# MDFahimAnjum/AliasFree-Diffusion-Models-PyTorch

Hardware: AMD Instinct MI355X
Metric: train_step_images_per_sec (higher is better)
Workload: dtype f32; 1 GPU; CIFAR-10 32x32x3 synthetic, UNet variant=3 (Config D), batch 256/GPU, T=1000, AdamW lr 3e-4, random-init weights (seed 42); global_batch=256, parallelism=dp1, hip_graph=True, launch_mode=lanes

## Files before the change

aliasfree-diffusion-models-pytorch_amd/_lib.py:

```python
import ctypes
import os
import re

_PKG = os.path.dirname(os.path.abspath(__file__))
_ROOT = os.path.dirname(_PKG)
HEADER = os.path.join(_ROOT, "include", "afd.h")
LIBPATH = os.environ.get("AFD_LIBPATH") or os.path.join(_PKG, "libafd_hip.so")

_CTYPES = {
    "int": ctypes.c_int, "long": ctypes.c_long, "float": ctypes.c_float, "double": ctypes.c_double,
    "size_t": ctypes.c_size_t,
}
_DECL = re.compile(r"^(int|size_t|const char\*)\s+(afd_\w+)\s*\(([^;]*?)\)\s*;", re.M | re.S)


def _strip_comments(src):
    return re.sub(r"/\*.*?\*/", " ", src, flags=re.S)


def parse_header(path=HEADER):
    out = {}
    for ret, name, args in _DECL.findall(_strip_comments(open(path).read())):
        argtypes = []
        args = " ".join(args.split())
        if args not in ("", "void"):
            for a in args.split(","):
                a = a.strip()
                if "*" in a or a.startswith("afd_stream_t"):
                    argtypes.append(ctypes.c_void_p)
                else:
                    base = a.split()[0] if not a.startswith("unsigned") else a
                    argtypes.append(_CTYPES[base])
        restype = {"int": ctypes.c_int, "size_t": ctypes.c_size_t, "const char*": ctypes.c_char_p}[ret]
        out[name] = (restype, argtypes)
    return out


_VALUE_RETURNING = {"afd_device_count", "afd_tok_supported", "afd_conv3x3_weight_kinds", "afd_conv_wgrad_form",
                    "afd_grad_sqnorm_n_partials"}


class AfdError(RuntimeError):
    pass


class _Lib:
    def __init__(self):
        if not os.path.exists(LIBPATH):
            raise AfdError(
                f"{LIBPATH} not found: build it with `python -c 'import __graft_entry__ as g; g.build()'` "
                "(hipcc --offload-arch=gfx950). There is no CPU/eager fallback.")
        self.cdll = ctypes.CDLL(LIBPATH)
        self.sigs = parse_header()
        for name, (restype, argtypes) in self.sigs.items():
            fn = getattr(self.cdll, name)
            fn.restype, fn.argtypes = restype, argtypes
            if restype is ctypes.c_int and name not in _VALUE_RETURNING:
                setattr(self, name, self._checked(name, fn))
            else:
                setattr(self, name, fn)

# ... 21 lines not shown
```

aliasfree-diffusion-models-pytorch_amd/csrc/bf3_wgrad.hip:

```cpp
#include <algorithm>
#include <cstdint>
#include <cstdlib>
#include "common.h"
#include "bf3_weights.h"

namespace afd {

using f32x4 = __attribute__((ext_vector_type(4))) float;
using u32x4 = __attribute__((ext_vector_type(4))) uint32_t;

template <int S, int BN_, int BK_> struct BwGeo {
  static constexpr int TP = 128, G8 = S / 8;
  static constexpr int IPT = S * S >= TP ? 1 : TP / (S * S);
  static constexpr int R = S * S >= TP ? TP / S : S;
  static constexpr int TPI = S * S >= TP ? S * S / TP : 1;
  static constexpr int IG = (R + 2) * G8, NG = IPT * IG;
  static constexpr int BK = BK_, BN = BN_;
  static constexpr int NR = (BN / 16) * (BK / 32), NSG = 8 / NR;
  static constexpr int TASKS = (BK / 16) * NG * 16, NE = (TASKS + 511) / 512;
  static constexpr int PIECE = (BK / 16) * NG * 16;
};

__device__ __forceinline__ uint32_t bf_pack(__bf16 lo, __bf16 hi) {
  return (uint32_t)__builtin_bit_cast(uint16_t, lo) | ((uint32_t)__builtin_bit_cast(uint16_t, hi) << 16);
// ... 426 lines not shown
  }
  float* ps = part + (long)blockIdx.x * 27 * N;
#pragma unroll
  for (int j = 0; j < 4; ++j)
#pragma unroll
    for (int t = 0; t < 27; ++t) {
      const float v = wave_sum_to_lane63(acc[j][t]);
      if (lane == 63) ps[((long)(t / 3) * N + n0 + j) * 3 + (t % 3)] = v;
    }
}

static int g_wgbf3_mode = 0;
void wgrad_bf3_set_mode(int m) { g_wgbf3_mode = m; }

static void wgrad_bf3_tile(int Cin, int Cout, long nt, int* bn, int* bk) {
  static const int force = [] { const char* e = getenv("AFD_WGB_TILE"); return e ? atoi(e) : 0; }();
  const bool can = Cout % 64 == 0 && Cin % 64 == 0;
  const bool big = force ? force >= 64 : nt * (Cout / 64) * (Cin / 64) >= 1024;
  if (can && big) { *bn = 64; *bk = 64; return; }
  *bn = (Cout % 64 == 0 && Cin % 64 && (force ? force >= 64 : true)) ? 64 : 32;
  *bk = (Cin % 64 == 0 && Cout % 64 && (force ? force >= 64 : true)) ? 64 : 32;
}

void wgrad_bf3_tile_for(int Cin, int Cout, long nt, int* bn, int* bk) { wgrad_bf3_tile(Cin, Cout, nt, bn, bk); }
static int g_wg_arith_bf3 = 0;
void wgrad_arith_set(int m) { g_wg_arith_bf3 = m; }
bool wgrad_arith_is_bf3() { return g_wg_arith_bf3 != 0; }

static long g_wgb_target = 256;
void wgrad_plan_target_set(long wgs) { g_wgb_target = wgs; }

int wgrad_bf3_plan(int B, int Cin, int Cout, int H, int W, int* tps, int* ntiles) {
  if (g_wgbf3_mode == 1) return 0;
  if (H != W || (W != 4 && W != 8 && W != 16 && W != 32)) return 0;
  if (Cin % 32 || Cout % 32) return 0;
  if ((long)B * H * W * (Cin > Cout ? Cin : Cout) >= (1L << 31)) return 0;
  const long nt = W == 4 ? (B + 7) / 8 : (W == 8 ? (B + 1) / 2 : (long)B * (H * W / 128));
  int BN, BK;
  wgrad_bf3_tile(Cin, Cout, W == 4 ? (B + 7) / 8 : (W == 8 ? (B + 1) / 2 : (long)B * (H * W / 128)), &BN, &BK);
  const long blocks = (long)(Cout / BN) * (Cin / BK);
  static const long env_target = [] { const char* e = getenv("AFD_WGB_TARGET"); return e ? atol(e) : 0L; }();
  const long target = env_target > 0 ? env_target : g_wgb_target;
  long s = target / blocks;
  if (s < 1) s = 1;
  if (s > nt) s = nt;
  const long c = (nt + s - 1) / s;
  if (g_wgbf3_mode != 2 && nt * blocks < 128) return 0;
  *tps = (int)c; *ntiles = (int)nt;
  return (int)((nt + c - 1) / c);
}

template <int S, int BN, int BK>
static void wgrad_bf3_launch_t(const float* x, const float* dy, float* part, int B, int Cin, int Cout, int tps, int nt, int splits,
                               hipStream_t s) {
  using G = BwGeo<S, BN, BK>;
  const size_t lds = std::max((size_t)3 * G::PIECE * 16, G::NSG > 1 ? sizeof(float) * G::NR * 72 * 64 : (size_t)0);
  (void)lds_opt_in(&wgrad_bf3<S, BN, BK>, lds);
  hipLaunchKernelGGL((wgrad_bf3<S, BN, BK>), dim3((unsigned)splits, (unsigned)((Cout / BN) * (Cin / BK))), dim3(512), lds, s, x, dy,
                     part, B, Cin, Cout, tps, nt);
}

template <int BN, int BK>
static void wgrad_bf3_s4_launch_t(const float* x, const float* dy, float* part, int B, int Cin, int Cout, int tps, int nt, int splits,
                                  hipStream_t s) {
  constexpr int NR = (BN / 16) * (BK / 32);
  const size_t lds = std::max((size_t)3 * (BK / 16) * 40 * 16 * 16, 8 / NR > 1 ? sizeof(float) * NR * 72 * 64 : (size_t)0);
  (void)lds_opt_in(&wgrad_bf3_s4<BN, BK>, lds);
  hipLaunchKernelGGL((wgrad_bf3_s4<BN, BK>), dim3((unsigned)splits, (unsigned)((Cout / BN) * (Cin / BK))), dim3(512), lds, s, x, dy, part, B,
                     Cin, Cout, tps, nt);
}

int wgrad_bf3(const float* x, const float* dy, float* part, int B, int Cin, int Cout, int H, int W, hipStream_t s) {
// ... 76 lines not shown
```

aliasfree-diffusion-models-pytorch_amd/csrc/conv.hip:

```cpp
#include <cstdlib>
#include <algorithm>
#include "common.h"

namespace afd {

using f32x16 = __attribute__((ext_vector_type(16))) float;

static inline int gs_grid(long total, int block = 256) {
  long g = (total + block - 1) / block;
  return (int)(g < 1 ? 1 : (g > 65536 ? 65536 : g));
}

template <int KS>
__global__ void conv_direct_fwd(const float* __restrict__ x, const float* __restrict__ w, const float* __restrict__ bias,
                                const float* __restrict__ res, float* __restrict__ y,
                                int Cin, int Cout, int H, int W, int act, long total) {
  constexpr int T = KS * KS, R = KS / 2;
  for (long i = blockIdx.x * (long)blockDim.x + threadIdx.x; i < total; i += (long)gridDim.x * blockDim.x) {
    const int xx = i % W, yy = (i / W) % H;
    const long bc = i / ((long)W * H);
    const int co = bc % Cout; const long b = bc / Cout;
    float acc = bias ? bias[co] : 0.f;
    for (int ci = 0; ci < Cin; ++ci) {
      const float* xp = x + (b * Cin + ci) * (long)H * W;
// ... 699 lines not shown
  }
  return fold_launch(d, nd, s);
}

bool pw_launch(const float* in, const float* w, const float* bias, const float* res, float* out, int B, int K, int N, int P,
               int act, bool dgrad, hipStream_t s);
void pw_set_mode(int m);
int wino_plan(int B, int K, int N, int H, int W);
int wino_conv(const float* x, const float* w, const float* bias, const float* res, float* y, float* U, int B, int K, int N, int H,
               int W, int act, bool dgrad, bool weights_ready, hipStream_t s);
void wino_set_mode(int m);
void wino_weights_launch(const float* w, float* Uf, float* Ud, int Cin, int Cout, int kinds, hipStream_t s);
bool bf3_ok(int B, int K, int N, int H, int W);
void bf3_set_mode(int m);
void direct_form_set(int m);
bool direct_form_is_bf3();
void h2_sk_set_mode(int m);
void h2_lds_set(int m);
void h2_skw_set(int m);
void wino_weights_batched_launch(const afd_wino_desc* descs, const int* wg_desc, int n_wg, hipStream_t s);
void wino_set_grid(int g);
int wgrad_wino_plan(int B, int Cin, int Cout, int H, int W, int* bn, int* bk, int* cps, int* nchunks);
int wgrad_bf3_plan(int B, int Cin, int Cout, int H, int W, int* tps, int* ntiles);
int wgrad_bf3(const float* x, const float* dy, float* part, int B, int Cin, int Cout, int H, int W, hipStream_t s);
void wgrad_bf3_set_mode(int m);
void wgrad_arith_set(int m);
void wgrad_plan_target_set(long wgs);
bool wgrad_arith_is_bf3();
int wgrad_h2(const float* x, const float* dy, float* part, int B, int Cin, int Cout, int H, int W, hipStream_t s);
int pw_wgrad_h2(const float* x, const float* dy, float* part, float* bias_part, int B, int Cin, int Cout, int L, hipStream_t s);
bool ends_fwd(const float* x, const float* w, const float* bias, const float* res, float* y, int B, int Cin, int Cout, int H, int W,
              int ksize, int act, hipStream_t s);
bool ends_dgrad(const float* dy, const float* w, float* dx, int B, int Cin, int Cout, int H, int W, int ksize, hipStream_t s);
void ends_set_mode(int m);
int wgrad_cin3_plan(int B, int Cin, int Cout, int H, int W);
int wgrad_cin3(const float* x, const float* dy, float* part, int B, int Cin, int Cout, int H, int W, hipStream_t s);
void pw_wgrad_bf3_set_mode(int m);
int pw_wgrad_bf3_plan(int B, int Cin, int Cout, int L, int* sps, int* nsteps, int* nr, int* nt);
int pw_wgrad_bf3(const float* x, const float* dy, float* part, float* bias_part, int B, int Cin, int Cout, int L, hipStream_t s);
int wgrad_wino(const float* x, const float* dy, float* part, int B, int Cin, int Cout, int H, int W, hipStream_t s);
void wgrad_wino_set_mode(int m);

static inline bool use_mfma(int K, int N, int H, int W, int PT) { return N >= 8 && tile_ok(H, W, PT); }

static int g_conv_path = 0;

template <int T, bool DGRAD>
static int launch_mfma(const float* x, const float* w, const float* bias, const float* res, float* y,
                       int B, int K, int N, int H, int W, int act, hipStream_t s) {
  constexpr int KC = (T == 9) ? 8 : 32;
// ... 73 lines not shown
  else
    hipLaunchKernelGGL((conv_wgrad_mfma<T, WNn, WCn, NPB, 4>), grid, dim3(256), lds, s, x, dy, part, bias_part, B, Cin, Cout, H, W, p.cps, p.nchunks, g);
}

template <int T, int NPB>
static void launch_wgrad_roles(const float* x, const float* dy, float* part, float* bp, int B, int Cin, int Cout, int H, int W,
                               const WgradPlan& p, const TileGeom& g, hipStream_t s) {
  if (p.wnn == 2 && p.wcn == 2) launch_wgrad<T, 2, 2, NPB>(x, dy, part, bp, B, Cin, Cout, H, W, p, g, s);
  else if (p.wnn == 2) launch_wgrad<T, 2, 1, NPB>(x, dy, part, bp, B, Cin, Cout, H, W, p, g, s);
  else if (p.wcn == 2) launch_wgrad<T, 1, 2, NPB>(x, dy, part, bp, B, Cin, Cout, H, W, p, g, s);
  else launch_wgrad<T, 1, 1, NPB>(x, dy, part, bp, B, Cin, Cout, H, W, p, g, s);
}

}
using namespace afd;

extern "C" {

int afd_debug_conv_path(int mode) {
  if (mode >= 92 && mode <= 93) { ends_set_mode(mode - 92); return AFD_OK; }
  if (mode >= 88 && mode <= 89) { pw_wgrad_bf3_set_mode(mode - 88); return AFD_OK; }
  if (mode >= 84 && mode <= 86) { wgrad_bf3_set_mode(mode - 84); return AFD_OK; }
  if (mode >= 48 && mode <= 49) { wgrad_plan_target_set(mode == 48 ? 256 : 160); return AFD_OK; }
  if (mode >= 59 && mode <= 63) { h2_lds_set(mode == 59 ? 4 : (mode == 60 ? 1 : (mode == 61 ? 0 : mode - 60))); return AFD_OK; }
  if (mode == 73) { h2_sk_set_mode(2); return AFD_OK; }
  if (mode >= 71 && mode <= 72) { h2_skw_set(mode - 70); return AFD_OK; }
  if (mode == 74) h2_skw_set(0);
  if (mode >= 74 && mode <= 75) { h2_sk_set_mode(mode - 74); return AFD_OK; }
  if (mode >= 78 && mode <= 79) { wgrad_arith_set(mode - 78); return AFD_OK; }
  if (mode >= 76 && mode <= 77) { direct_form_set(mode - 76); return AFD_OK; }
  if (mode >= 80 && mode <= 82) { bf3_set_mode(mode - 80); return AFD_OK; }
  if (mode >= 8 && mode <= 10) { pw_set_mode(mode - 8); return AFD_OK; }
  if (mode >= 100000 && mode < 200000) { wino_set_grid(mode - 100000); return AFD_OK; }
  if (mode >= 96 && mode <= 98) { wgrad_wino_set_mode(mode - 96); return AFD_OK; }
  if (mode >= 64 && mode <= 70) { wino_set_mode(mode - 64); return AFD_OK; }
  if (mode >= 32 && mode <= 34) { g_wgrad_nw = mode == 32 ? 4 : (mode == 33 ? 8 : 0); return AFD_OK; }
  AFD_REQUIRE(mode >= 0 && mode <= 2, "afd_debug_conv_path: mode must be 0 (auto), 1 (big tile), 2 (split-K tile), 8..10 (1x1 streaming auto/off/forced), 32..34 (wgrad waves 4/8/auto), 64..69 (Winograd fwd/dgrad auto/off/forced shapes) or 96..98 (Winograd wgrad auto/off/forced)");
  g_conv_path = mode;
  return AFD_OK;
}

int afd_conv_fwd(const float* x, const float* w, const float* bias, const float* res, float* y,
                 int B, int Cin, int Cout, int H, int W, int ksize, int act, afd_stream_t st) {
  AFD_REQUIRE(x && w && y && B > 0 && Cin > 0 && Cout > 0 && H > 0 && W > 0, "afd_conv_fwd: bad argument");
  AFD_REQUIRE(ksize == 1 || ksize == 3, "afd_conv_fwd: ksize %d not in {1,3}", ksize);
  AFD_REQUIRE(act == 0 || act == 1, "afd_conv_fwd: act must be 0 or 1");
// ... 98 lines not shown
  size_t slabs = wgrad_plan(B, Cin, Cout, H, W, ksize).slabs;
  if (ksize == 3) {
    int bn, bk, cps, nch;
    const size_t ws = (size_t)wgrad_wino_plan(B, Cin, Cout, H, W, &bn, &bk, &cps, &nch);
    if (ws > slabs) slabs = ws;
    const size_t wb = (size_t)wgrad_bf3_plan(B, Cin, Cout, H, W, &cps, &nch);
    if (wb > slabs) slabs = wb;
    const size_t wc = (size_t)wgrad_cin3_plan(B, Cin, Cout, H, W);
    if (wc > slabs) slabs = wc;
  }
  const size_t need = slabs * ((size_t)Cout * Cin * ksize * ksize + Cout);
  const size_t direct = (size_t)B * Cout;
  return std::max(pw, sizeof(float) * (need > direct ? need : direct));
}

int afd_conv_wgrad_form(int B, int Cin, int Cout, int H, int W, int ksize) {
  if (B <= 0 || Cin <= 0 || Cout <= 0 || H <= 0 || W <= 0) return 0;
  int a, b, c, d;
  if (ksize == 1) return pw_wgrad_bf3_plan(B, Cin, Cout, H * W, &a, &b, &c, &d) ? (wgrad_arith_is_bf3() ? 2 : 4) : 0;
  if (ksize != 3) return 0;
  if (wgrad_bf3_plan(B, Cin, Cout, H, W, &a, &b)) return wgrad_arith_is_bf3() ? 2 : 4;
  if (wgrad_cin3_plan(B, Cin, Cout, H, W)) return 3;
  return wgrad_wino_plan(B, Cin, Cout, H, W, &a, &b, &c, &d) ? 1 : 0;
}

static int conv_wgrad_impl(const float* x, const float* dy, float* dw, float* dbias, int B, int Cin, int Cout, int H, int W,
                           int ksize, int accumulate, void* workspace, FoldSink* sink, hipStream_t s, const char* who) {
  AFD_REQUIRE(x && dy && dw && B > 0 && Cin > 0 && Cout > 0 && H > 0 && W > 0, "%s: bad argument", who);
  AFD_REQUIRE(ksize == 1 || ksize == 3, "%s: ksize %d not in {1,3}", who, ksize);
  const int T = ksize * ksize;
  const TileGeom g = make_geom(H, W, 64, ksize == 3 ? 1 : 0);
  int rc = AFD_OK;
  const bool vec = aligned16(x) && aligned16(dy);
  if (ksize == 3 && !dbias && workspace) {
    float* part = static_cast<float*>(workspace);
    int slabs = !vec ? 0 : (wgrad_arith_is_bf3() ? wgrad_bf3(x, dy, part, B, Cin, Cout, H, W, s) : wgrad_h2(x, dy, part, B, Cin, Cout, H, W, s));
    if (!slabs) slabs = wgrad_cin3(x, dy, part, B, Cin, Cout, H, W, s);
    if (!slabs && vec) slabs = wgrad_wino(x, dy, part, B, Cin, Cout, H, W, s);
    if (slabs) {
      const long n = (long)Cout * Cin * 9;
      rc = launch_wgrad_reduce(part, dw, n, slabs, nullptr, nullptr, 0, accumulate, 9, s, sink);
      return rc != AFD_OK ? rc : check_launch(who);
    }
  }
  if (ksize == 1 && workspace && vec) {
    int a, b, c, d;
// ... 54 lines not shown
```

aliasfree-diffusion-models-pytorch_amd/csrc/h2_wgrad.hip:

```cpp
#include <algorithm>
#include <cstdint>
#include <cstdlib>
#include "common.h"
#include "h2_common.h"

namespace afd {

using f32x4 = __attribute__((ext_vector_type(4))) float;
using u32x4 = __attribute__((ext_vector_type(4))) uint32_t;

template <int S, int BN_, int BK_> struct HwGeo {
  static constexpr int TP = 128, G8 = S / 8;
  static constexpr int IPT = S * S >= TP ? 1 : TP / (S * S);
  static constexpr int R = S * S >= TP ? TP / S : S;
  static constexpr int TPI = S * S >= TP ? S * S / TP : 1;
  static constexpr int IG = (R + 2) * G8, NG = IPT * IG;
  static constexpr int BK = BK_, BN = BN_;
  static constexpr int NR = (BN / 16) * (BK / 32), NSG = 8 / NR;
  static constexpr int TASKS = (BK / 16) * NG * 16, NE = (TASKS + 511) / 512;
  static constexpr int PIECE = (BK / 16) * NG * 16;
};

__device__ __forceinline__ uint32_t h_pack(_Float16 lo, _Float16 hi) {
  return (uint32_t)__builtin_bit_cast(uint16_t, lo) | ((uint32_t)__builtin_bit_cast(uint16_t, hi) << 16);
}

template <int NR, int NSG>
__device__ __forceinline__ void hw_finish(f32x4 (&acc)[2][9], float unscale_x, float unscale_d, uint8_t* smem_raw, float* __restrict__ part,
                                          int split, int role, int sg, int lane, int n0w, int k0w, int N, int K) {
  const int l15 = lane & 15, kgl = lane >> 4;
#pragma unroll
  for (int ks = 0; ks < 2; ++ks)
#pragma unroll
    for (int t = 0; t < 9; ++t) acc[ks][t] = (acc[ks][t] * unscale_x) * unscale_d;
  if (NSG > 1) {
    float* red = reinterpret_cast<float*>(smem_raw);
#pragma unroll 1
    for (int g = 1; g < NSG; ++g) {
      __syncthreads();
      if (sg == g) {
#pragma unroll
        for (int ks = 0; ks < 2; ++ks)
// ... 41 lines not shown
#pragma unroll
      for (int t = 0; t < 3; ++t)
#pragma unroll
        for (int tx = 0; tx < 3; ++tx)
          acc[ks][ty * 3 + tx] = __builtin_amdgcn_mfma_f32_16x16x32_f16(af[tx][TA[t]], bc[TB[t]], acc[ks][ty * 3 + tx], 0, 0, 0);
    }
    __builtin_amdgcn_sched_barrier(0);
    bc[0] = bn[0]; bc[1] = bn[1];
  }
}

__device__ __forceinline__ void hw_rescale(f32x4 (&acc)[2][9], float& s, float m) {
  const float sn = fminf(s, h2_scale_for(m));
  if (sn != s) {
    const float f = sn * h2_inv_pow2(s);
#pragma unroll
    for (int ks = 0; ks < 2; ++ks)
#pragma unroll
      for (int t = 0; t < 9; ++t) acc[ks][t] *= f;
    s = sn;
  }
}

template <int S, int BN, int BK>
__global__ __launch_bounds__(512, 1) void wgrad_h2(const float* __restrict__ x, const float* __restrict__ dy, float* __restrict__ part,
                                                    int B, int K, int N, int tiles_per_split, int ntiles) {
  using G = HwGeo<S, BN, BK>;
  constexpr int HW = S * S, G8 = G::G8, NG = G::NG, NE = G::NE, PIECE = G::PIECE, NSG = G::NSG;
  extern __shared__ __attribute__((aligned(16))) uint8_t smem_raw[];
  h8* Xs = reinterpret_cast<h8*>(smem_raw);
  float* wmax = reinterpret_cast<float*>(smem_raw + (size_t)2 * PIECE * 16);
  const int tid = threadIdx.x, lane = tid & 63, wv = tid >> 6, l15 = lane & 15, kgl = lane >> 4;
  const int role = wv % G::NR, sg = wv / G::NR;
  const int ns = role % (BN / 16), kh = role / (BN / 16);
  const int nkb = blockIdx.y, nbk = N / G::BN;
  const int n0 = (nkb % nbk) * G::BN, k0 = (nkb / nbk) * G::BK;
  const int split = blockIdx.x;
  const int tbeg = split * tiles_per_split, tend = min(ntiles, tbeg + tiles_per_split);

  int s_off[NE], s_rr[NE];
#pragma unroll
  for (int e = 0; e < NE; ++e) {
    const int t = tid + 512 * e;
    s_rr[e] = -1; s_off[e] = 0;
    if (t < G::TASKS) {
      const int c16 = t & 15, g = (t >> 4) % NG, ksub = t / (16 * NG);
      const int i = g / G::IG, rem = g - i * G::IG, rr = rem / G8, c8 = rem - rr * G8;
      s_rr[e] = rr | (i << 8);
      s_off[e] = (i * K + ksub * 16 + c16) * HW + (rr - 1) * S + c8 * 8;
    }
  }
  float xr[NE][8];
  auto x_fetch = [&](int tile) {
    const int img0 = G::IPT > 1 ? tile * G::IPT : tile / G::TPI;
    const int row0 = G::IPT > 1 ? 0 : (tile % G::TPI) * G::R;
    const float* xb = x + ((long)img0 * K + k0) * HW + row0 * S;
#pragma unroll
    for (int e = 0; e < NE; ++e) {
      const int rr = s_rr[e] & 255, i = s_rr[e] >> 8, yy = row0 + rr - 1;
      const bool ok = s_rr[e] >= 0 && yy >= 0 && yy < S && img0 + i < B;
      const float4* p = reinterpret_cast<const float4*>(xb + (ok ? s_off[e] : 0));
      const float4 a = ok ? p[0] : make_float4(0.f, 0.f, 0.f, 0.f), b = ok ? p[1] : make_float4(0.f, 0.f, 0.f, 0.f);
      xr[e][0] = a.x; xr[e][1] = a.y; xr[e][2] = a.z; xr[e][3] = a.w; xr[e][4] = b.x; xr[e][5] = b.y; xr[e][6] = b.z; xr[e][7] = b.w;
    }
  };
  auto x_amax = [&]() {
    float m = 0.f;
#pragma unroll
    for (int e = 0; e < NE; ++e)
#pragma unroll
      for (int j = 0; j < 8; ++j) m = fmaxf(m, fabsf(xr[e][j]));
    m = wave_amax(m);
    if (lane == 0) wmax[wv] = m;
  };
  auto x_commit = [&](float s) {
#pragma unroll
    for (int e = 0; e < NE; ++e) {
      if (s_rr[e] < 0) continue;
      h8 p0, p1;
      h2_split8(xr[e], s, p0, p1);
      const int t = tid + 512 * e;
      Xs[t] = p0; Xs[PIECE + t] = p1;
    }
  };

  float dv[10];
  const float* dyw = dy + (long)(n0 + 16 * ns + l15) * HW;
  auto d_fetch = [&](int tile, int step) {
    const int img0 = G::IPT > 1 ? tile * G::IPT : tile / G::TPI;
    const int row0 = G::IPT > 1 ? 0 : (tile % G::TPI) * G::R;
    const int pg = 4 * step + kgl;
    const int i = pg / (G::R * G8), rem = pg - i * (G::R * G8), r = rem / G8, c8 = rem - r * G8;
    const bool ok = img0 + i < B;
    const float* p = dyw + (long)(img0 + i) * N * HW + (row0 + r) * S + c8 * 8;
    const float4 a = ok ? reinterpret_cast<const float4*>(p)[0] : make_float4(0.f, 0.f, 0.f, 0.f);
    const float4 b = ok ? reinterpret_cast<const float4*>(p)[1] : make_float4(0.f, 0.f, 0.f, 0.f);
    dv[1] = a.x; dv[2] = a.y; dv[3] = a.z; dv[4] = a.w; dv[5] = b.x; dv[6] = b.y; dv[7] = b.z; dv[8] = b.w;
    dv[0] = (G8 > 1 && ok && c8 > 0) ? p[-1] : 0.f;
    dv[9] = (G8 > 1 && ok && c8 < G8 - 1) ? p[8] : 0.f;
  };

  f32x4 acc[2][9];
#pragma unroll
  for (int ks = 0; ks < 2; ++ks)
#pragma unroll
    for (int t = 0; t < 9; ++t) acc[ks][t] = f32x4{0.f, 0.f, 0.f, 0.f};

  const int brec0 = ((2 * kh) * NG) * 16 + l15;
  auto b_group = [&](int step) {
    const int pg = 4 * step + kgl;
    const int i = pg / (G::R * G8), rem = pg - i * (G::R * G8), r = rem / G8, c8 = rem - r * G8;
    return i * G::IG + (r + 1) * G8 + c8;
  };

  float sx = __uint_as_float(kH2ScaleCapBits), sd = sx;
  if (tbeg < tend) { x_fetch(tbeg); d_fetch(tbeg, sg); }
  for (int tile = tbeg; tile < tend; ++tile) {
    x_amax();
    __syncthreads();
    {
      float m = wmax[0];
#pragma unroll
      for (int q = 1; q < 8; ++q) m = fmaxf(m, wmax[q]);
      hw_rescale(acc, sx, m);
    }
    x_commit(sx);
    __syncthreads();
    if (tile + 1 < tend) x_fetch(tile + 1);
#pragma unroll 1
    for (int step = sg; step < 4; step += NSG) {
      {
        float m = 0.f;
#pragma unroll
        for (int j = 0; j < 10; ++j) m = fmaxf(m, fabsf(dv[j]));
        hw_rescale(acc, sd, wave_amax(m));
      }
      _Float16 pc[2][10];
#pragma unroll
      for (int j = 0; j < 10; ++j) h2_split(dv[j], sd, pc[0][j], pc[1][j]);
      h8 af[3][2];
#pragma unroll
      for (int p = 0; p < 2; ++p) {
        u32x4 e0, e1, e2;
#pragma unroll
        for (int q = 0; q < 4; ++q) {
          e0[q] = h_pack(pc[p][2 * q + 2], pc[p][2 * q + 3]);
          e1[q] = h_pack(pc[p][2 * q + 1], pc[p][2 * q + 2]);
          e2[q] = h_pack(pc[p][2 * q], pc[p][2 * q + 1]);
        }
        af[0][p] = __builtin_bit_cast(h8, e0); af[1][p] = __builtin_bit_cast(h8, e1); af[2][p] = __builtin_bit_cast(h8, e2);
      }
      if (step + NSG < 4) d_fetch(tile, step + NSG); else if (tile + 1 < tend) d_fetch(tile + 1, sg);

      hw_step(acc, af, Xs, PIECE, brec0 + b_group(step) * 16, NG * 16, -G8 * 16, 0, G8 * 16);
    }
  }

  hw_finish<G::NR, NSG>(acc, h2_inv_pow2(sx), h2_inv_pow2(sd), smem_raw, part, split, role, sg, lane, n0 + 16 * ns, k0 + 32 * kh, N, K);
}


template <int BN, int BK>
__global__ __launch_bounds__(512, 1) void wgrad_h2_s4(const float* __restrict__ x, const float* __restrict__ dy, float* __restrict__ part,
                                                       int B, int K, int N, int tiles_per_split, int ntiles) {
  constexpr int NR = (BN / 16) * (BK / 32), NSG = 8 / NR, NG = 40, PIECE = (BK / 16) * NG * 16, TASKS = 8 * BK;
  extern __shared__ __attribute__((aligned(16))) uint8_t smem_raw[];
  h8* Xs = reinterpret_cast<h8*>(smem_raw);
  float* wmax = reinterpret_cast<float*>(smem_raw + (size_t)2 * PIECE * 16);
  const int tid = threadIdx.x, lane = tid & 63, wv = tid >> 6, l15 = lane & 15, kgl = lane >> 4;
  const int role = wv % NR, sg = wv / NR;
  const int ns = role % (BN / 16), kh = role / (BN / 16);
  const int nkb = blockIdx.y, nbk = N / BN;
  const int n0 = (nkb % nbk) * BN, k0 = (nkb / nbk) * BK;
  const int split = blockIdx.x;
  const int tbeg = split * tiles_per_split, tend = min(ntiles, tbeg + tiles_per_split);

  const bool has_task = tid < TASKS;
  const int ti = tid / BK, tc = tid % BK;
  float xr[16];
  auto x_fetch = [&](int tile) {
    const int img = tile * 8 + ti;
    const bool ok = has_task && img < B;
    const float4* p = reinterpret_cast<const float4*>(x + ((long)(ok ? img : 0) * K + k0 + tc) * 16);
#pragma unroll
    for (int q = 0; q < 4; ++q) {
      const float4 v = ok ? p[q] : make_float4(0.f, 0.f, 0.f, 0.f);
      xr[4 * q] = v.x; xr[4 * q + 1] = v.y; xr[4 * q + 2] = v.z; xr[4 * q + 3] = v.w;
    }
  };
  auto x_amax = [&]() {
    float m = 0.f;
#pragma unroll
    for (int j = 0; j < 16; ++j) m = fmaxf(m, fabsf(xr[j]));
    m = wave_amax(m);
    if (lane == 0) wmax[wv] = m;
  };
  auto x_commit = [&](float s) {
    if (!has_task) return;
    _Float16 pc[2][16];
#pragma unroll
    for (int j = 0; j < 16; ++j) h2_split(xr[j], s, pc[0][j], pc[1][j]);
    const _Float16 Z = (_Float16)0.f;
    const int rec = (((tc >> 4) * 8 + ti) * 5) * 16 + (tc & 15);
#pragma unroll
    for (int p = 0; p < 2; ++p) {
      h8 a0, a1, o0, o1, o2;
#pragma unroll
      for (int j = 0; j < 8; ++j) {
        a0[j] = pc[p][j]; a1[j] = pc[p][8 + j]; o1[j] = pc[p][4 + j];
        o0[j] = j < 4 ? Z : pc[p][j - 4];
        o2[j] = j < 4 ? pc[p][12 + j] : Z;
      }
      h8* d = Xs + p * PIECE + rec;
      d[0] = a0; d[16] = a1; d[32] = o0; d[48] = o1; d[64] = o2;
    }
  };

  float dv[8];
  const float* dyw = dy + (long)(n0 + 16 * ns + l15) * 16;
  auto d_fetch = [&](int tile, int step) {
    const int img = tile * 8 + 2 * step + (kgl >> 1);
    const bool ok = img < B;
    const float4* p = reinterpret_cast<const float4*>(dyw + (long)(ok ? img : 0) * N * 16 + (kgl & 1) * 8);
    const float4 a = ok ? p[0] : make_float4(0.f, 0.f, 0.f, 0.f), b = ok ? p[1] : make_float4(0.f, 0.f, 0.f, 0.f);
    dv[0] = a.x; dv[1] = a.y; dv[2] = a.z; dv[3] = a.w; dv[4] = b.x; dv[5] = b.y; dv[6] = b.z; dv[7] = b.w;
  };

  f32x4 acc[2][9];
#pragma unroll
  for (int ks = 0; ks < 2; ++ks)
#pragma unroll
    for (int t = 0; t < 9; ++t) acc[ks][t] = f32x4{0.f, 0.f, 0.f, 0.f};
  const int brec0 = ((2 * kh) * NG) * 16 + l15;

  float sx = __uint_as_float(kH2ScaleCapBits), sd = sx;
  if (!has_task) {
#pragma unroll
    for (int j = 0; j < 16; ++j) xr[j] = 0.f;
  }
  if (tbeg < tend) { x_fetch(tbeg); d_fetch(tbeg, sg); }
  for (int tile = tbeg; tile < tend; ++tile) {
    x_amax();
    __syncthreads();
    {
      float m = wmax[0];
#pragma unroll
      for (int q = 1; q < 8; ++q) m = fmaxf(m, wmax[q]);
      hw_rescale(acc, sx, m);
    }
    x_commit(sx);
    __syncthreads();
    if (tile + 1 < tend) x_fetch(tile + 1);
#pragma unroll 1
    for (int step = sg; step < 4; step += NSG) {
      {
        float m = 0.f;
#pragma unroll
        for (int j = 0; j < 8; ++j) m = fmaxf(m, fabsf(dv[j]));
        hw_rescale(acc, sd, wave_amax(m));
      }
      _Float16 pc[2][8];
#pragma unroll
      for (int j = 0; j < 8; ++j) h2_split(dv[j], sd, pc[0][j], pc[1][j]);
      const _Float16 Z = (_Float16)0.f;
      h8 af[3][2];
#pragma unroll
      for (int p = 0; p < 2; ++p)
#pragma unroll
        for (int j = 0; j < 8; ++j) {
          af[1][p][j] = pc[p][j];
// ... 120 lines not shown
      for (int i = 0; i < NT; ++i) {
#pragma unroll
        for (int j = 0; j < 2; ++j)
#pragma unroll
          for (int rg = 0; rg < 4; ++rg) acc[i][j][rg] += red[(rl * (NT * 9) + (i * 2 + j) * 4 + rg) * 64 + lane];
        bsum[i] += red[(rl * (NT * 9) + NT * 8 + i) * 64 + lane];
      }
    }
  }
  if (wp != 0) return;
  float* ps = part + (long)split * N * K;
#pragma unroll
  for (int i = 0; i < NT; ++i)
#pragma unroll
    for (int j = 0; j < 2; ++j)
#pragma unroll
      for (int rg = 0; rg < 4; ++rg) ps[(long)(n0 + 16 * i + 4 * kgl + rg) * K + k0 + 16 * j + l15] = acc[i][j][rg];
  if (bias_part && k0 == 0 && kgl == 0) {
#pragma unroll
    for (int i = 0; i < NT; ++i) bias_part[(long)split * N + n0 + 16 * i + l15] = bsum[i];
  }
}

int wgrad_bf3_plan(int B, int Cin, int Cout, int H, int W, int* tps, int* ntiles);
void wgrad_bf3_tile_for(int Cin, int Cout, long nt, int* bn, int* bk);

template <int S, int BN, int BK>
static void wgrad_h2_launch_t(const float* x, const float* dy, float* part, int B, int Cin, int Cout, int tps, int nt, int splits,
                              hipStream_t s) {
  using G = HwGeo<S, BN, BK>;
  const size_t lds = std::max((size_t)2 * G::PIECE * 16 + 32, G::NSG > 1 ? sizeof(float) * G::NR * 72 * 64 : (size_t)0);
  (void)lds_opt_in(&wgrad_h2<S, BN, BK>, lds);
  hipLaunchKernelGGL((wgrad_h2<S, BN, BK>), dim3((unsigned)splits, (unsigned)((Cout / BN) * (Cin / BK))), dim3(512), lds, s, x, dy,
                     part, B, Cin, Cout, tps, nt);
}

template <int BN, int BK>
static void wgrad_h2_s4_launch_t(const float* x, const float* dy, float* part, int B, int Cin, int Cout, int tps, int nt, int splits,
                                 hipStream_t s) {
  constexpr int NR = (BN / 16) * (BK / 32);
  const size_t lds = std::max((size_t)2 * (BK / 16) * 40 * 16 * 16 + 32, 8 / NR > 1 ? sizeof(float) * NR * 72 * 64 : (size_t)0);
  (void)lds_opt_in(&wgrad_h2_s4<BN, BK>, lds);
  hipLaunchKernelGGL((wgrad_h2_s4<BN, BK>), dim3((unsigned)splits, (unsigned)((Cout / BN) * (Cin / BK))), dim3(512), lds, s, x, dy, part, B,
                     Cin, Cout, tps, nt);
}

int wgrad_h2(const float* x, const float* dy, float* part, int B, int Cin, int Cout, int H, int W, hipStream_t s) {
  int tps, nt;
  const int splits = wgrad_bf3_plan(B, Cin, Cout, H, W, &tps, &nt);
  if (!splits) return 0;
  int bn_, bk_;
  wgrad_bf3_tile_for(Cin, Cout, nt, &bn_, &bk_);
  const bool n64 = bn_ == 64, k64 = bk_ == 64;
#define AFD_WGH(S_)                                                                                      \
  if (n64 && k64) wgrad_h2_launch_t<S_, 64, 64>(x, dy, part, B, Cin, Cout, tps, nt, splits, s);          \
  else if (n64) wgrad_h2_launch_t<S_, 64, 32>(x, dy, part, B, Cin, Cout, tps, nt, splits, s);            \
  else if (k64) wgrad_h2_launch_t<S_, 32, 64>(x, dy, part, B, Cin, Cout, tps, nt, splits, s);            \
  else wgrad_h2_launch_t<S_, 32, 32>(x, dy, part, B, Cin, Cout, tps, nt, splits, s)
  if (W == 32) { AFD_WGH(32); } else if (W == 16) { AFD_WGH(16); } else if (W == 8) { AFD_WGH(8); }
  else if (n64 && k64) wgrad_h2_s4_launch_t<64, 64>(x, dy, part, B, Cin, Cout, tps, nt, splits, s);
  else if (n64) wgrad_h2_s4_launch_t<64, 32>(x, dy, part, B, Cin, Cout, tps, nt, splits, s);
  else if (k64) wgrad_h2_s4_launch_t<32, 64>(x, dy, part, B, Cin, Cout, tps, nt, splits, s);
  else wgrad_h2_s4_launch_t<32, 32>(x, dy, part, B, Cin, Cout, tps, nt, splits, s);
#undef AFD_WGH
  return splits;
}


int pw_wgrad_bf3_plan(int B, int Cin, int Cout, int L, int* sps, int* nsteps, int* nr, int* nt);
int pw_wgrad_h2(const float* x, const float* dy, float* part, float* bias_part, int B, int Cin, int Cout, int L, hipStream_t s) {
  int sps, st, NR, NT;
  const int splits = pw_wgrad_bf3_plan(B, Cin, Cout, L, &sps, &st, &NR, &NT);
  if (!splits) return 0;
  const int roles = (Cout / (16 * NT)) * (Cin / 32);
  const size_t lds = 8 / NR > 1 ? sizeof(float) * NR * NT * 9 * 64 : 0;
  const dim3 grid((unsigned)splits, (unsigned)(roles / NR));
  if (NT == 3) hipLaunchKernelGGL(pw_wgrad_h2<3>, grid, dim3(512), lds, s, x, dy, part, bias_part, B, Cin, Cout, L, sps, st, NR);
  else hipLaunchKernelGGL(pw_wgrad_h2<2>, grid, dim3(512), lds, s, x, dy, part, bias_part, B, Cin, Cout, L, sps, st, NR);
  return splits;
}

}
```

include/afd.h:

```cpp
#ifndef AFD_H_
#define AFD_H_

#include <stddef.h>
#include <stdint.h>

#ifdef __cplusplus
extern "C" {
#endif

#define AFD_OK 0
#define AFD_EINVAL 1
#define AFD_ELAUNCH 2
#define AFD_MAX_TAPS 15

typedef void* afd_stream_t;

const char* afd_version(void);
const char* afd_last_error(void);
int afd_device_count(void);

int afd_lowpass_kernel(double omega_c, int N, int has_beta, double beta, float* taps_out);

int afd_filt_up2_fwd(const float* x, float* y, int B, int C, int H, int W, long x_bstride, long y_bstride,
                     const float* taps, int N, afd_stream_t stream);
// ... 22 lines not shown
                     const float* taps_up, const float* taps_down, int N,
                     void* workspace, float* gn_partials, afd_stream_t stream);

int afd_groupnorm1_fwd(const float* x, float* y, float* stats_out, int B, int C, int HW, float eps,
                       const float* gamma, const float* beta, const float* res, int act, const float* emb,
                       afd_stream_t stream);
int afd_debug_norm_path(int mode);
int afd_groupnorm1_bwd(const float* x, const float* dy, const float* stats, int B, int C, int HW,
                       const float* gamma, const float* beta, const float* res, int act,
                       float* dx, float* dres, float* dgamma_dbeta_partial , float* demb ,
                       int have_partials ,
                       float* dgamma , float* dbeta , int accumulate, afd_stream_t stream);
int afd_colsum(const float* in, float* out, int rows, int cols, int accumulate, afd_stream_t stream);
int afd_colsum_strided(const float* in, long row_stride, float* out, int rows, int cols, int accumulate, afd_stream_t stream);
int afd_colsum2(const float* in, float* out_a, float* out_b, int rows, int C, int accumulate, afd_stream_t stream);

int afd_debug_conv_path(int mode);
int afd_conv_fwd(const float* x, const float* w, const float* bias, const float* res, float* y,
                 int B, int Cin, int Cout, int H, int W, int ksize, int act, afd_stream_t stream);
int afd_conv_dgrad(const float* dy, const float* w, float* dx,
                   int B, int Cin, int Cout, int H, int W, int ksize, afd_stream_t stream);
size_t afd_conv_wgrad_workspace_bytes(int B, int Cin, int Cout, int H, int W, int ksize);
int afd_conv_wgrad_form(int B, int Cin, int Cout, int H, int W, int ksize);
int afd_conv_wgrad(const float* x, const float* dy, float* dw, float* dbias ,
                   int B, int Cin, int Cout, int H, int W, int ksize, int accumulate,
                   void* workspace, afd_stream_t stream);

typedef struct afd_fold_desc {
  const float* part;
  float* dst;
  long n;
  long stride;
  long inner, rstride;
  int splits;
  int accumulate;
} afd_fold_desc;
int afd_fold_batched(const afd_fold_desc* descs, int n, afd_stream_t stream);
int afd_conv_wgrad_partials(const float* x, const float* dy, float* dw, float* dbias ,
                            int B, int Cin, int Cout, int H, int W, int ksize, int accumulate,
                            void* workspace, afd_fold_desc* folds_out, int* n_folds, afd_stream_t stream);

size_t afd_conv3x3_wino_workspace_bytes(int B, int Cin, int Cout, int H, int W, int dgrad);
int afd_conv3x3_wino_weights(const float* w, float* u_fwd, float* u_dgrad, int Cin, int Cout, int kinds, afd_stream_t stream);
int afd_conv3x3_weight_kinds(int B, int Cin, int Cout, int H, int W);
typedef struct afd_wino_desc {
  const float* w;
// ... 324 lines not shown
```

Baseline: 38980 images/s.

## Add four-wave workgroup variants for split-fp16 3x3 weight-gradient kernels

```diff
diff --git a/aliasfree-diffusion-models-pytorch_amd/_lib.py b/aliasfree-diffusion-models-pytorch_amd/_lib.py
--- a/aliasfree-diffusion-models-pytorch_amd/_lib.py
+++ b/aliasfree-diffusion-models-pytorch_amd/_lib.py
@@ -36,7 +36,7 @@
     return out
 
 
-_VALUE_RETURNING = {"afd_device_count", "afd_tok_supported", "afd_conv3x3_weight_kinds", "afd_conv_wgrad_form",
+_VALUE_RETURNING = {"afd_device_count", "afd_tok_supported", "afd_conv3x3_weight_kinds", "afd_conv_wgrad_form", "afd_conv_wgrad3_plan",
                     "afd_grad_sqnorm_n_partials"}
 
 
diff --git a/aliasfree-diffusion-models-pytorch_amd/csrc/bf3_wgrad.hip b/aliasfree-diffusion-models-pytorch_amd/csrc/bf3_wgrad.hip
--- a/aliasfree-diffusion-models-pytorch_amd/csrc/bf3_wgrad.hip
+++ b/aliasfree-diffusion-models-pytorch_amd/csrc/bf3_wgrad.hip
@@ -472,7 +472,6 @@
   *bk = (Cin % 64 == 0 && Cout % 64 && (force ? force >= 64 : true)) ? 64 : 32;
 }
 
-void wgrad_bf3_tile_for(int Cin, int Cout, long nt, int* bn, int* bk) { wgrad_bf3_tile(Cin, Cout, nt, bn, bk); }
 static int g_wg_arith_bf3 = 0;
 void wgrad_arith_set(int m) { g_wg_arith_bf3 = m; }
 bool wgrad_arith_is_bf3() { return g_wg_arith_bf3 != 0; }
@@ -480,24 +479,56 @@
 static long g_wgb_target = 256;
 void wgrad_plan_target_set(long wgs) { g_wgb_target = wgs; }
 
-int wgrad_bf3_plan(int B, int Cin, int Cout, int H, int W, int* tps, int* ntiles) {
+static int g_wg_waves_mode = 0;
+void wgrad_waves_set(int m) { g_wg_waves_mode = m; }
+static constexpr int kWg4RuleMask = 7;
+static bool wgrad_four_waves(int BN, int BK) {
+  if (g_wg_arith_bf3) return false;
+  static const int force = [] { const char* e = getenv("AFD_WGB_WAVES"); return e ? atoi(e) : 0; }();
+  static const int mask = [] { const char* e = getenv("AFD_WGB_W4"); return e ? atoi(e) : kWg4RuleMask; }();
+  if (force == 4 || force == 8) return force == 4;
+  if (g_wg_waves_mode) return g_wg_waves_mode >= 2;
+  const int kind = BN == 64 && BK == 64 ? 1 : (BN == 64 || BK == 64 ? 2 : 4);
+  return (mask & kind) != 0;
+}
+
+int wgrad_plan_full(int B, int Cin, int Cout, int H, int W, int* tps, int* ntiles, int* bn, int* bk, int* nw) {
   if (g_wgbf3_mode == 1) return 0;
   if (H != W || (W != 4 && W != 8 && W != 16 && W != 32)) return 0;
   if (Cin % 32 || Cout % 32) return 0;
   if ((long)B * H * W * (Cin > Cout ? Cin : Cout) >= (1L << 31)) return 0;
   const long nt = W == 4 ? (B + 7) / 8 : (W == 8 ? (B + 1) / 2 : (long)B * (H * W / 128));
   int BN, BK;
-  wgrad_bf3_tile(Cin, Cout, W == 4 ? (B + 7) / 8 : (W == 8 ? (B + 1) / 2 : (long)B * (H * W / 128)), &BN, &BK);
+  wgrad_bf3_tile(Cin, Cout, nt, &BN, &BK);
+  if (g_wg_waves_mode >= 3 && !g_wg_arith_bf3) {
+    if (g_wg_waves_mode == 3 && Cout % 64 == 0) { BN = 64; BK = 32; }
+    else if (g_wg_waves_mode == 4 && Cin % 64 == 0) { BN = 32; BK = 64; }
+    else if (g_wg_waves_mode == 5) { BN = 32; BK = 32; }
+  }
   const long blocks = (long)(Cout / BN) * (Cin / BK);
-  static const long env_target = [] { const char* e = getenv("AFD_WGB_TARGET"); return e ? atol(e) : 0L; }();
+  const char* et = getenv("AFD_WGB_TARGET");
+  const long env_target = et ? atol(et) : 0L;
   const long target = env_target > 0 ? env_target : g_wgb_target;
   long s = target / blocks;
   if (s < 1) s = 1;
   if (s > nt) s = nt;
+  if (g_wgbf3_mode != 2 && nt * blocks < 128) return 0;
+  int NW = 8;
+  if (wgrad_four_waves(BN, BK)) {
+    static const long target4 = [] { const char* e = getenv("AFD_WGB_TARGET4"); return e ? atol(e) : 0L; }();
+    NW = 4;
+    if (BN == 64 && BK == 64) BK = 32;
+    const long s4 = (target4 > 0 ? target4 : target) / ((long)(Cout / BN) * (Cin / BK));
+    if (s4 < s) s = s4 < 1 ? 1 : s4;
+  }
   const long c = (nt + s - 1) / s;
-  if (g_wgbf3_mode != 2 && nt * blocks < 128) return 0;
-  *tps = (int)c; *ntiles = (int)nt;
+  *tps = (int)c; *ntiles = (int)nt; *bn = BN; *bk = BK; *nw = NW;
   return (int)((nt + c - 1) / c);
+}
+
+int wgrad_bf3_plan(int B, int Cin, int Cout, int H, int W, int* tps, int* ntiles) {
+  int bn, bk, nw;
+  return wgrad_plan_full(B, Cin, Cout, H, W, tps, ntiles, &bn, &bk, &nw);
 }
 
 template <int S, int BN, int BK>
diff --git a/aliasfree-diffusion-models-pytorch_amd/csrc/conv.hip b/aliasfree-diffusion-models-pytorch_amd/csrc/conv.hip
--- a/aliasfree-diffusion-models-pytorch_amd/csrc/conv.hip
+++ b/aliasfree-diffusion-models-pytorch_amd/csrc/conv.hip
@@ -745,10 +745,12 @@
 void wino_set_grid(int g);
 int wgrad_wino_plan(int B, int Cin, int Cout, int H, int W, int* bn, int* bk, int* cps, int* nchunks);
 int wgrad_bf3_plan(int B, int Cin, int Cout, int H, int W, int* tps, int* ntiles);
+int wgrad_plan_full(int B, int Cin, int Cout, int H, int W, int* tps, int* ntiles, int* bn, int* bk, int* nw);
 int wgrad_bf3(const float* x, const float* dy, float* part, int B, int Cin, int Cout, int H, int W, hipStream_t s);
 void wgrad_bf3_set_mode(int m);
 void wgrad_arith_set(int m);
 void wgrad_plan_target_set(long wgs);
+void wgrad_waves_set(int m);
 bool wgrad_arith_is_bf3();
 int wgrad_h2(const float* x, const float* dy, float* part, int B, int Cin, int Cout, int H, int W, hipStream_t s);
 int pw_wgrad_h2(const float* x, const float* dy, float* part, float* bias_part, int B, int Cin, int Cout, int L, hipStream_t s);
@@ -868,6 +870,7 @@
   if (mode >= 88 && mode <= 89) { pw_wgrad_bf3_set_mode(mode - 88); return AFD_OK; }
   if (mode >= 84 && mode <= 86) { wgrad_bf3_set_mode(mode - 84); return AFD_OK; }
   if (mode >= 48 && mode <= 49) { wgrad_plan_target_set(mode == 48 ? 256 : 160); return AFD_OK; }
+  if (mode >= 50 && mode <= 55) { wgrad_waves_set(mode - 50); return AFD_OK; }
   if (mode >= 59 && mode <= 63) { h2_lds_set(mode == 59 ? 4 : (mode == 60 ? 1 : (mode == 61 ? 0 : mode - 60))); return AFD_OK; }
   if (mode == 73) { h2_sk_set_mode(2); return AFD_OK; }
   if (mode >= 71 && mode <= 72) { h2_skw_set(mode - 70); return AFD_OK; }
@@ -1012,6 +1015,12 @@
   if (wgrad_bf3_plan(B, Cin, Cout, H, W, &a, &b)) return wgrad_arith_is_bf3() ? 2 : 4;
   if (wgrad_cin3_plan(B, Cin, Cout, H, W)) return 3;
   return wgrad_wino_plan(B, Cin, Cout, H, W, &a, &b, &c, &d) ? 1 : 0;
+}
+
+int afd_conv_wgrad3_plan(int B, int Cin, int Cout, int H, int W, int* info) {
+  if (!info || B <= 0 || Cin <= 0 || Cout <= 0 || H <= 0 || W <= 0) return 0;
+  for (int i = 0; i < 5; ++i) info[i] = 0;
+  return wgrad_plan_full(B, Cin, Cout, H, W, &info[0], &info[1], &info[2], &info[3], &info[4]);
 }
 
 static int conv_wgrad_impl(const float* x, const float* dy, float* dw, float* dbias, int B, int Cin, int Cout, int H, int W,
diff --git a/aliasfree-diffusion-models-pytorch_amd/csrc/h2_wgrad.hip b/aliasfree-diffusion-models-pytorch_amd/csrc/h2_wgrad.hip
--- a/aliasfree-diffusion-models-pytorch_amd/csrc/h2_wgrad.hip
+++ b/aliasfree-diffusion-models-pytorch_amd/csrc/h2_wgrad.hip
@@ -9,15 +9,16 @@
 using f32x4 = __attribute__((ext_vector_type(4))) float;
 using u32x4 = __attribute__((ext_vector_type(4))) uint32_t;
 
-template <int S, int BN_, int BK_> struct HwGeo {
+template <int S, int BN_, int BK_, int NW_ = 8> struct HwGeo {
   static constexpr int TP = 128, G8 = S / 8;
   static constexpr int IPT = S * S >= TP ? 1 : TP / (S * S);
   static constexpr int R = S * S >= TP ? TP / S : S;
   static constexpr int TPI = S * S >= TP ? S * S / TP : 1;
   static constexpr int IG = (R + 2) * G8, NG = IPT * IG;
-  static constexpr int BK = BK_, BN = BN_;
-  static constexpr int NR = (BN / 16) * (BK / 32), NSG = 8 / NR;
-  static constexpr int TASKS = (BK / 16) * NG * 16, NE = (TASKS + 511) / 512;
+  static constexpr int BK = BK_, BN = BN_, NW = NW_, NT = 64 * NW;
+  static constexpr int NR = (BN / 16) * (BK / 32), NSG = NW / NR;
+  static_assert(NR <= NW && NSG * NR == NW && NSG <= 4, "block and waves per workgroup do not fit");
+  static constexpr int TASKS = (BK / 16) * NG * 16, NE = (TASKS + NT - 1) / NT;
   static constexpr int PIECE = (BK / 16) * NG * 16;
 };
 
@@ -105,11 +106,11 @@
   }
 }
 
-template <int S, int BN, int BK>
-__global__ __launch_bounds__(512, 1) void wgrad_h2(const float* __restrict__ x, const float* __restrict__ dy, float* __restrict__ part,
+template <int S, int BN, int BK, int NW>
+__global__ __launch_bounds__(64 * NW, 8 / NW) void wgrad_h2(const float* __restrict__ x, const float* __restrict__ dy, float* __restrict__ part,
                                                     int B, int K, int N, int tiles_per_split, int ntiles) {
-  using G = HwGeo<S, BN, BK>;
-  constexpr int HW = S * S, G8 = G::G8, NG = G::NG, NE = G::NE, PIECE = G::PIECE, NSG = G::NSG;
+  using G = HwGeo<S, BN, BK, NW>;
+  constexpr int HW = S * S, G8 = G::G8, NG = G::NG, NE = G::NE, PIECE = G::PIECE, NSG = G::NSG, NT = G::NT;
   extern __shared__ __attribute__((aligned(16))) uint8_t smem_raw[];
   h8* Xs = reinterpret_cast<h8*>(smem_raw);
   float* wmax = reinterpret_cast<float*>(smem_raw + (size_t)2 * PIECE * 16);
@@ -124,7 +125,7 @@
   int s_off[NE], s_rr[NE];
 #pragma unroll
   for (int e = 0; e < NE; ++e) {
-    const int t = tid + 512 * e;
+    const int t = tid + NT * e;
     s_rr[e] = -1; s_off[e] = 0;
     if (t < G::TASKS) {
       const int c16 = t & 15, g = (t >> 4) % NG, ksub = t / (16 * NG);
@@ -162,7 +163,7 @@
       if (s_rr[e] < 0) continue;
       h8 p0, p1;
       h2_split8(xr[e], s, p0, p1);
-      const int t = tid + 512 * e;
+      const int t = tid + NT * e;
       Xs[t] = p0; Xs[PIECE + t] = p1;
     }
   };
@@ -204,7 +205,7 @@
     {
       float m = wmax[0];
 #pragma unroll
-      for (int q = 1; q < 8; ++q) m = fmaxf(m, wmax[q]);
+      for (int q = 1; q < NW; ++q) m = fmaxf(m, wmax[q]);
       hw_rescale(acc, sx, m);
     }
     x_commit(sx);
@@ -243,10 +244,12 @@
 }
 
 
-template <int BN, int BK>
-__global__ __launch_bounds__(512, 1) void wgrad_h2_s4(const float* __restrict__ x, const float* __restrict__ dy, float* __restrict__ part,
+template <int BN, int BK, int NW>
+__global__ __launch_bounds__(64 * NW, 8 / NW) void wgrad_h2_s4(const float* __restrict__ x, const float* __restrict__ dy, float* __restrict__ part,
                                                        int B, int K, int N, int tiles_per_split, int ntiles) {
-  constexpr int NR = (BN / 16) * (BK / 32), NSG = 8 / NR, NG = 40, PIECE = (BK / 16) * NG * 16, TASKS = 8 * BK;
+  constexpr int NR = (BN / 16) * (BK / 32), NSG = NW / NR, NG = 40, PIECE = (BK / 16) * NG * 16, TASKS = 8 * BK, NT = 64 * NW;
+  constexpr int NE = (TASKS + NT - 1) / NT;
+  static_assert(NR <= NW && NSG * NR == NW && NSG <= 4, "block and waves per workgroup do not fit");
   extern __shared__ __attribute__((aligned(16))) uint8_t smem_raw[];
   h8* Xs = reinterpret_cast<h8*>(smem_raw);
   float* wmax = reinterpret_cast<float*>(smem_raw + (size_t)2 * PIECE * 16);
@@ -258,44 +261,53 @@
   const int split = blockIdx.x;
   const int tbeg = split * tiles_per_split, tend = min(ntiles, tbeg + tiles_per_split);
 
-  const bool has_task = tid < TASKS;
-  const int ti = tid / BK, tc = tid % BK;
-  float xr[16];
+  auto has_task = [&](int e) { return tid + NT * e < TASKS; };
+  float xr[NE][16];
   auto x_fetch = [&](int tile) {
-    const int img = tile * 8 + ti;
-    const bool ok = has_task && img < B;
-    const float4* p = reinterpret_cast<const float4*>(x + ((long)(ok ? img : 0) * K + k0 + tc) * 16);
-#pragma unroll
-    for (int q = 0; q < 4; ++q) {
-      const float4 v = ok ? p[q] : make_float4(0.f, 0.f, 0.f, 0.f);
-      xr[4 * q] = v.x; xr[4 * q + 1] = v.y; xr[4 * q + 2] = v.z; xr[4 * q + 3] = v.w;
+#pragma unroll
+    for (int e = 0; e < NE; ++e) {
+      const int t = tid + NT * e, ti = t / BK, tc = t % BK;
+      const int img = tile * 8 + ti;
+      const bool ok = has_task(e) && img < B;
+      const float4* p = reinterpret_cast<const float4*>(x + ((long)(ok ? img : 0) * K + k0 + tc) * 16);
+#pragma unroll
+      for (int q = 0; q < 4; ++q) {
+        const float4 v = ok ? p[q] : make_float4(0.f, 0.f, 0.f, 0.f);
+        xr[e][4 * q] = v.x; xr[e][4 * q + 1] = v.y; xr[e][4 * q + 2] = v.z; xr[e][4 * q + 3] = v.w;
+      }
     }
   };
   auto x_amax = [&]() {
     float m = 0.f;
 #pragma unroll
-    for (int j = 0; j < 16; ++j) m = fmaxf(m, fabsf(xr[j]));
+    for (int e = 0; e < NE; ++e)
+#pragma unroll
+      for (int j = 0; j < 16; ++j) m = fmaxf(m, fabsf(xr[e][j]));
     m = wave_amax(m);
     if (lane == 0) wmax[wv] = m;
   };
   auto x_commit = [&](float s) {
-    if (!has_task) return;
-    _Float16 pc[2][16];
-#pragma unroll
-    for (int j = 0; j < 16; ++j) h2_split(xr[j], s, pc[0][j], pc[1][j]);
-    const _Float16 Z = (_Float16)0.f;
-    const int rec = (((tc >> 4) * 8 + ti) * 5) * 16 + (tc & 15);
-#pragma unroll
-    for (int p = 0; p < 2; ++p) {
-      h8 a0, a1, o0, o1, o2;
-#pragma unroll
-      for (int j = 0; j < 8; ++j) {
-        a0[j] = pc[p][j]; a1[j] = pc[p][8 + j]; o1[j] = pc[p][4 + j];
-        o0[j] = j < 4 ? Z : pc[p][j - 4];
-        o2[j] = j < 4 ? pc[p][12 + j] : Z;
-      }
-      h8* d = Xs + p * PIECE + rec;
-      d[0] = a0; d[16] = a1; d[32] = o0; d[48] = o1; d[64] = o2;
+#pragma unroll
+    for (int e = 0; e < NE; ++e) {
+      if (!has_task(e)) continue;
+      const int t = tid + NT * e, ti = t / BK, tc = t % BK;
+      _Float16 pc[2][16];
+#pragma unroll
+      for (int j = 0; j < 16; ++j) h2_split(xr[e][j], s, pc[0][j], pc[1][j]);
+      const _Float16 Z = (_Float16)0.f;
+      const int rec = (((tc >> 4) * 8 + ti) * 5) * 16 + (tc & 15);
+#pragma unroll
+      for (int p = 0; p < 2; ++p) {
+        h8 a0, a1, o0, o1, o2;
+#pragma unroll
+        for (int j = 0; j < 8; ++j) {
+          a0[j] = pc[p][j]; a1[j] = pc[p][8 + j]; o1[j] = pc[p][4 + j];
+          o0[j] = j < 4 ? Z : pc[p][j - 4];
+          o2[j] = j < 4 ? pc[p][12 + j] : Z;
+        }
+        h8* d = Xs + p * PIECE + rec;
+        d[0] = a0; d[16] = a1; d[32] = o0; d[48] = o1; d[64] = o2;
+      }
     }
   };
 
@@ -317,10 +329,10 @@
   const int brec0 = ((2 * kh) * NG) * 16 + l15;
 
   float sx = __uint_as_float(kH2ScaleCapBits), sd = sx;
-  if (!has_task) {
-#pragma unroll
-    for (int j = 0; j < 16; ++j) xr[j] = 0.f;
-  }
+#pragma unroll
+  for (int e = 0; e < NE; ++e)
+#pragma unroll
+    for (int j = 0; j < 16; ++j) xr[e][j] = 0.f;
   if (tbeg < tend) { x_fetch(tbeg); d_fetch(tbeg, sg); }
   for (int tile = tbeg; tile < tend; ++tile) {
     x_amax();
@@ -328,7 +340,7 @@
     {
       float m = wmax[0];
 #pragma unroll
-      for (int q = 1; q < 8; ++q) m = fmaxf(m, wmax[q]);
+      for (int q = 1; q < NW; ++q) m = fmaxf(m, wmax[q]);
       hw_rescale(acc, sx, m);
     }
     x_commit(sx);
@@ -495,47 +507,56 @@
   }
 }
 
-int wgrad_bf3_plan(int B, int Cin, int Cout, int H, int W, int* tps, int* ntiles);
-void wgrad_bf3_tile_for(int Cin, int Cout, long nt, int* bn, int* bk);
-
-template <int S, int BN, int BK>
+int wgrad_plan_full(int B, int Cin, int Cout, int H, int W, int* tps, int* ntiles, int* bn, int* bk, int* nw);
+
+template <int S, int BN, int BK, int NW>
 static void wgrad_h2_launch_t(const float* x, const float* dy, float* part, int B, int Cin, int Cout, int tps, int nt, int splits,
                               hipStream_t s) {
-  using G = HwGeo<S, BN, BK>;
+  using G = HwGeo<S, BN, BK, NW>;
   const size_t lds = std::max((size_t)2 * G::PIECE * 16 + 32, G::NSG > 1 ? sizeof(float) * G::NR * 72 * 64 : (size_t)0);
-  (void)lds_opt_in(&wgrad_h2<S, BN, BK>, lds);
-  hipLaunchKernelGGL((wgrad_h2<S, BN, BK>), dim3((unsigned)splits, (unsigned)((Cout / BN) * (Cin / BK))), dim3(512), lds, s, x, dy,
+  (void)lds_opt_in(&wgrad_h2<S, BN, BK, NW>, lds);
+  hipLaunchKernelGGL((wgrad_h2<S, BN, BK, NW>), dim3((unsigned)splits, (unsigned)((Cout / BN) * (Cin / BK))), dim3(G::NT), lds, s, x, dy,
                      part, B, Cin, Cout, tps, nt);
 }
 
-template <int BN, int BK>
+template <int BN, int BK, int NW>
 static void wgrad_h2_s4_launch_t(const float* x, const float* dy, float* part, int B, int Cin, int Cout, int tps, int nt, int splits,
                                  hipStream_t s) {
   constexpr int NR = (BN / 16) * (BK / 32);
-  const size_t lds = std::max((size_t)2 * (BK / 16) * 40 * 16 * 16 + 32, 8 / NR > 1 ? sizeof(float) * NR * 72 * 64 : (size_t)0);
-  (void)lds_opt_in(&wgrad_h2_s4<BN, BK>, lds);
-  hipLaunchKernelGGL((wgrad_h2_s4<BN, BK>), dim3((unsigned)splits, (unsigned)((Cout / BN) * (Cin / BK))), dim3(512), lds, s, x, dy, part, B,
-                     Cin, Cout, tps, nt);
+  const size_t lds = std::max((size_t)2 * (BK / 16) * 40 * 16 * 16 + 32, NW / NR > 1 ? sizeof(float) * NR * 72 * 64 : (size_t)0);
+  (void)lds_opt_in(&wgrad_h2_s4<BN, BK, NW>, lds);
+  hipLaunchKernelGGL((wgrad_h2_s4<BN, BK, NW>), dim3((unsigned)splits, (unsigned)((Cout / BN) * (Cin / BK))), dim3(64 * NW), lds, s, x, dy,
+                     part, B, Cin, Cout, tps, nt);
+}
+
+template <int S, int BN, int BK, int NW>
+static void wgrad_h2_form_t(const float* x, const float* dy, float* part, int B, int Cin, int Cout, int tps, int nt, int splits, hipStream_t s) {
+  if constexpr (S == 0) wgrad_h2_s4_launch_t<BN, BK, NW>(x, dy, part, B, Cin, Cout, tps, nt, splits, s);
+  else wgrad_h2_launch_t<S, BN, BK, NW>(x, dy, part, B, Cin, Cout, tps, nt, splits, s);
+}
+
+template <int S>
+static void wgrad_h2_map_t(const float* x, const float* dy, float* part, int B, int Cin, int Cout, int tps, int nt, int splits, int bn, int bk,
+                           int nw, hipStream_t s) {
+  const bool n64 = bn == 64, k64 = bk == 64;
+  if (nw == 4) {
+    if (n64) wgrad_h2_form_t<S, 64, 32, 4>(x, dy, part, B, Cin, Cout, tps, nt, splits, s);
+    else if (k64) wgrad_h2_form_t<S, 32, 64, 4>(x, dy, part, B, Cin, Cout, tps, nt, splits, s);
+    else wgrad_h2_form_t<S, 32, 32, 4>(x, dy, part, B, Cin, Cout, tps, nt, splits, s);
+  } else if (n64 && k64) wgrad_h2_form_t<S, 64, 64, 8>(x, dy, part, B, Cin, Cout, tps, nt, splits, s);
+  else if (n64) wgrad_h2_form_t<S, 64, 32, 8>(x, dy, part, B, Cin, Cout, tps, nt, splits, s);
+  else if (k64) wgrad_h2_form_t<S, 32, 64, 8>(x, dy, part, B, Cin, Cout, tps, nt, splits, s);
+  else wgrad_h2_form_t<S, 32, 32, 8>(x, dy, part, B, Cin, Cout, tps, nt, splits, s);
 }
 
 int wgrad_h2(const float* x, const float* dy, float* part, int B, int Cin, int Cout, int H, int W, hipStream_t s) {
-  int tps, nt;
-  const int splits = wgrad_bf3_plan(B, Cin, Cout, H, W, &tps, &nt);
+  int tps, nt, bn, bk, nw;
+  const int splits = wgrad_plan_full(B, Cin, Cout, H, W, &tps, &nt, &bn, &bk, &nw);
   if (!splits) return 0;
-  int bn_, bk_;
-  wgrad_bf3_tile_for(Cin, Cout, nt, &bn_, &bk_);
-  const bool n64 = bn_ == 64, k64 = bk_ == 64;
-#define AFD_WGH(S_)                                                                                      \
-  if (n64 && k64) wgrad_h2_launch_t<S_, 64, 64>(x, dy, part, B, Cin, Cout, tps, nt, splits, s);          \
-  else if (n64) wgrad_h2_launch_t<S_, 64, 32>(x, dy, part, B, Cin, Cout, tps, nt, splits, s);            \
-  else if (k64) wgrad_h2_launch_t<S_, 32, 64>(x, dy, part, B, Cin, Cout, tps, nt, splits, s);            \
-  else wgrad_h2_launch_t<S_, 32, 32>(x, dy, part, B, Cin, Cout, tps, nt, splits, s)
-  if (W == 32) { AFD_WGH(32); } else if (W == 16) { AFD_WGH(16); } else if (W == 8) { AFD_WGH(8); }
-  else if (n64 && k64) wgrad_h2_s4_launch_t<64, 64>(x, dy, part, B, Cin, Cout, tps, nt, splits, s);
-  else if (n64) wgrad_h2_s4_launch_t<64, 32>(x, dy, part, B, Cin, Cout, tps, nt, splits, s);
-  else if (k64) wgrad_h2_s4_launch_t<32, 64>(x, dy, part, B, Cin, Cout, tps, nt, splits, s);
-  else wgrad_h2_s4_launch_t<32, 32>(x, dy, part, B, Cin, Cout, tps, nt, splits, s);
-#undef AFD_WGH
+  if (W == 32) wgrad_h2_map_t<32>(x, dy, part, B, Cin, Cout, tps, nt, splits, bn, bk, nw, s);
+  else if (W == 16) wgrad_h2_map_t<16>(x, dy, part, B, Cin, Cout, tps, nt, splits, bn, bk, nw, s);
+  else if (W == 8) wgrad_h2_map_t<8>(x, dy, part, B, Cin, Cout, tps, nt, splits, bn, bk, nw, s);
+  else wgrad_h2_map_t<0>(x, dy, part, B, Cin, Cout, tps, nt, splits, bn, bk, nw, s);
   return splits;
 }
 
diff --git a/include/afd.h b/include/afd.h
--- a/include/afd.h
+++ b/include/afd.h
@@ -68,6 +68,7 @@
                    int B, int Cin, int Cout, int H, int W, int ksize, afd_stream_t stream);
 size_t afd_conv_wgrad_workspace_bytes(int B, int Cin, int Cout, int H, int W, int ksize);
 int afd_conv_wgrad_form(int B, int Cin, int Cout, int H, int W, int ksize);
+int afd_conv_wgrad3_plan(int B, int Cin, int Cout, int H, int W, int* info);
 int afd_conv_wgrad(const float* x, const float* dy, float* dw, float* dbias ,
                    int B, int Cin, int Cout, int H, int W, int ksize, int accumulate,
                    void* workspace, afd_stream_t stream);
```

After: 39800 images/s, median of 6. 1.02x the previous value.
